# grero/HMMSpikeSorter.jl

Hardware: AMD Instinct MI355X
Metric: Msamples/sec (Viterbi + forward-backward), K=4 L=60 HMM (higher is better)
Workload: dtype f64; 1 GPU; K=4 L=60 HMM (reference N=4, K=60: 237 states), 10000000-sample single channel per GPU: one Viterbi decode + one Baum-Welch E-step (forward-backward + sufficient statistics + M-step finish); channels=1, samples_per_channel=10000000, states=237, engine=wave, block=4928, halo=295, chains=2030, seed=1234, pooled_allreduce=False

## Files before the change

hmmspikesorter.jl_amd/csrc/wave_estep.hip:

```cpp
#include <cmath>
#include <type_traits>

#include "fastmath.h"
#include "wave_common.h"

namespace hmmsort {

constexpr double kLn2 = 6.93147180559945286227e-01;
typedef double wg_d4 __attribute__((ext_vector_type(4)));

__device__ __forceinline__ double scale_of(double v, double s)
{
    return v > 0.0 ? s + (double)ilogb(v) * kLn2 : -INFINITY;
}

template <int N>
struct FIn {
    double y;
    double R[N];
};

template <int N>
__device__ __forceinline__ void excl_sums(const double (&t)[N], double (&out)[N])
{
// ... 82 lines not shown
        d.y = (yc + tb)[li];
#pragma unroll
        for (int a = 0; a < N; a++) d.R[a] = (Rc + (int64_t)a * T + tb)[li];
    };
    int rs = (1 + lane) % RB, ws = (L + 1 + lane) % RB;
    auto run = [&](const FIn<N> &d, int off, auto mode_tag) {
        constexpr int MODE = decltype(mode_tag)::value;
        const int nact = n_total - off < W ? n_total - off : W;
        const bool live = lane < nact;
        const int64_t tb = tinit + 1 + off;
        const int64_t t = tb + lane;
        const double sc0 = KC[0];
        double v[N], E[N + 1];
        double e = -INFINITY;
#pragma unroll
        for (int a = 0; a < N; a++) {
            if (LOGDL) {
                v[a] = 1.0;
                E[a] = live ? DLs[a * (RB + 1) + rs] + sc0 : -INFINITY;
                e = fmax(e, E[a]);
            } else {
                v[a] = live ? DLv[a * (RB + 1) + rs] : 0.0;
                E[a] = DLs[a * (RB + 1) + rs] + sc0;
                e = fmax(e, scale_of(v[a], E[a]));
            }
        }
        const double dd = d.y - KC[1];
        const double q0 = -((dd * dd) * KC[2]);
        float fa = live ? (float)(sc0 + q0) : 0.0f;
        float fb = live ? (float)(e + q0) : -INFINITY;
        scan_maxplus_f32(fa, fb);
        const float Mf = (float)M;
        const float Mtf = fmaxf(Mf + fa, fb);
        const double Mt = (double)Mtf;
        const double Mprev = (double)lane_prevf(Mtf, Mf);
        const double ref = Mt - q0;
        E[N] = (Mprev + sc0) - ref;
#pragma unroll
        for (int a = 0; a < N; a++) E[a] = v[a] > 0.0 ? fmin(E[a] - ref, 700.0) : -INFINITY;
        fexp_n<N + 1>(E);
        const double E0 = E[N];
        double Ea[N];
        double al = E0 * KC[3], be = 0.0;
#pragma unroll
        for (int a = 0; a < N; a++) {
            Ea[a] = LOGDL ? E[a] : v[a] * E[a];
            be = __builtin_fma(Ea[a], KC[KPEND + a], be);
        }
        al = live ? al : 1.0;
        be = live ? be : 0.0;
        scan_linear(al, be);
        const double xt = __builtin_fma(al, x, be);
        const double xprev = lane_prev(xt, x);
        const double einv = KC[4];
        const double base = (xprev * E0) * einv;
        double u[N];
        if (UC) {
            double tb_[N], ex[N];
#pragma unroll
            for (int a = 0; a < N; a++) tb_[a] = Ea[a] * einv;
            excl_sums<N>(tb_, ex);
#pragma unroll
            for (int a = 0; a < N; a++) u[a] = __builtin_fma(ex[a], KC[KCPX + a], base * KC[KCP0 + a]);
        } else {
#pragma unroll
            for (int a = 0; a < N; a++) {
                double su = base * KC[KCP0 + a];
#pragma unroll
                for (int b = 0; b < N; b++)
                    if (b != a) su = __builtin_fma(Ea[b] * einv, KC[KCPX + a * N + b], su);
                u[a] = su;
                __builtin_amdgcn_sched_barrier(0);
            }
        }
        const int wsl = live ? ws : RB;
        if (LOGDL) {
            double lu[N];
#pragma unroll
            for (int a = 0; a < N; a++) lu[a] = u[a];
            flog_n<N>(lu);
#pragma unroll
            for (int a = 0; a < N; a++) DLs[a * (RB + 1) + wsl] = ((ref + KC[KSC + a]) + d.R[a]) + (u[a] > 0.0 ? lu[a] : -INFINITY);
        } else {
#pragma unroll
            for (int a = 0; a < N; a++) {
                DLv[a * (RB + 1) + wsl] = u[a];
                DLs[a * (RB + 1) + wsl] = (ref + KC[KSC + a]) + d.R[a];
            }
        }
        if (MODE == 1) {
            const double la0 = Mt + flog(xt);
            *(live ? FAc + tb + lane : trash + lane) = la0;
            *(live ? FRc + tb + lane : trash + 64 + lane) = ref;
#pragma unroll
            for (int a = 0; a < N; a++) *(live ? FVc + (int64_t)a * T + tb + lane : trash + 64 * (2 + a) + lane) = u[a];
        }
        if (MODE == 2) {
            if (live && t >= tc - L && t < tc) {
                const int64_t jj = t - (tc - L);
#pragma unroll
                for (int a = 0; a < N; a++) rec[1 + jj * (N + 1) + a] = u[a];
                rec[1 + jj * (N + 1) + N] = ref;
                if (t == tc - 1) rec[0] = Mt + flog(xt);
            }
        }
        x = wave_bcast(xt, nact - 1);
        M = wave_bcast(Mt, nact - 1);
        const int ee = x > 0.0 ? ilogb(x) : 0;
        if (ee >= 32 || ee <= -32) {
            const double Mx = M + (double)ee * kLn2, Mn = (double)(float)Mx;
            x = ldexp(x, -ee) * fexp(Mx - Mn);
            M = Mn;
        }
        rs += W; rs = rs >= RB ? rs - RB : rs;
        ws += W; ws = ws >= RB ? ws - RB : ws;
    };
    auto sweep = [&](int from, int to, auto mode_tag) {
        FIn<N> buf[D];
#pragma unroll
        for (int i = 0; i < D; i++) load(buf[i], from + i * W);
        int off = from;
        for (; off + D * W <= to; off += D * W) {
#pragma unroll
            for (int i = 0; i < D; i++) {
                run(buf[i], off + i * W, mode_tag);
                load(buf[i], off + (i + D) * W);
            }
        }
#pragma unroll
        for (int i = 0; i < D; i++)
            if (off + i * W < to) run(buf[i], off + i * W, mode_tag);
    };
    const int n_warm = c == 0 ? 0 : g.Hw - 1;
    const int n_rec = ((L + W - 1) / W) * W < n_warm ? ((L + W - 1) / W) * W : n_warm;
    if (n_warm - n_rec > 0) sweep(0, n_warm - n_rec, std::integral_constant<int, 0>());
    if (n_rec > 0) sweep(n_warm - n_rec, n_warm, std::integral_constant<int, 2>());
    sweep(n_warm, n_total, std::integral_constant<int, 1>());
}

template <int N>
struct BIn {
    double y1, y0;
    double w2;
    double R[N];
    double fv[N];
    double fref, la0;
};

constexpr int bwd_yring(int ft) { return ft <= 2 ? 256 : 512; }

#ifndef HS_BWD_W4
#define HS_BWD_W4 2
#endif
template <int N, bool UC, int FT = 0, bool GS = false>
__global__ __launch_bounds__(64, N <= 4 ? HS_BWD_W4 : 1) void kw_bwd(WaveGeom g, const WaveConst *__restrict__ cst,
                                                            const double *__restrict__ y,
                                                            const double *__restrict__ Rf,
                                                            const double *__restrict__ FA0,
                                                            const double *__restrict__ FV,
                                                            const double *__restrict__ FREF,
                                                            const double *__restrict__ fpre,
                                                            const double *__restrict__ W2,
                                                            double *__restrict__ rho, double *__restrict__ partS,
                                                            double *__restrict__ Zc, double *__restrict__ bpre,
                                                            double *__restrict__ bown, double *__restrict__ yhead,
                                                            double *__restrict__ trash, double *__restrict__ partG,
                                                            double *__restrict__ gsil)
{
    constexpr bool FUSE = FT > 0;
    static_assert(!GS || !FUSE, "the silent posterior is stored by the unfused sweep");
    static_assert(!FUSE || (N >= 3 && N <= 8), "the fused statistics are written for delayed copies of 3-8 rings");
    static_assert(!FUSE || N > 4 || FT == 1, "3-4 rings: one tile of 64 lags");
    constexpr int NPc = N <= 4 ? 4 : 8, NSc = 16 / NPc, LPT = 16 * NSc;
    constexpr int RPAD = NPc == 4 ? 1 : 2;
    constexpr int RGROWS = 128 + 8 * RPAD;
    constexpr int YM = bwd_yring(FT);
    constexpr int NACC = FT <= 1 ? 2 : FT;
#ifndef HS_BWD_D4
#define HS_BWD_D4 2
#endif
    constexpr int D = N <= 4 ? HS_BWD_D4 : (N <= 8 ? 2 : 1);
    constexpr int KSC = 4, KCP0 = 4 + N, KPEND = 4 + 2 * N, KCPX = 4 + 3 * N, KSIZE = 4 + 3 * N + N * N;
    extern __shared__ double lds[];
    const int L = g.L, W = g.W, RB = g.RB, B = g.B;
    double *KC = lds, *DLv = lds + KSIZE, *DLs = lds + KSIZE + N * (RB + 1);
    const int lane = threadIdx.x;
    const int cg = blockIdx.x, ch = cg / g.nch, c = cg % g.nch;
    const int64_t T = g.T;
    const int64_t tc = (int64_t)c * B;
    const int nc = (int)((T - tc) < B ? (T - tc) : B);
    const int64_t tend = tc + nc, tstar = tend - 1;
    const int64_t te = (tend + g.He) < T ? (tend + g.He) : T;
    const double *yc = y + (int64_t)ch * T;
    const double *Rc = Rf + (int64_t)ch * N * T;
    const double *FAc = FA0 + (int64_t)ch * T, *FRc = FREF + (int64_t)ch * T, *FVc = FV + (int64_t)ch * N * T;
    double *rhoc = rho + (int64_t)ch * N * T;
    const double *W2c = W2 + (int64_t)ch * T;
    const int64_t FR = 1 + (int64_t)L * (N + 1);
    const double la0pre = c > 0 ? fpre[cg * FR] : 0.0;
    double *recp = bpre + cg * FR, *reco = bown + cg * FR;
    double *yh = yhead + (int64_t)ch * (N * L + 2);

    for (int i = lane; i < N * (RB + 1); i += 64) DLv[i] = 1.0;
    for (int i = lane; i < RB + 1; i += 64) DLs[i] = 0.0;
    double *YY = DLs + (RB + 1), *RG = YY + YM;
    const int lk = lane >> 4, lj = lane & 15, gla = lj % NPc, glsft = lj / NPc;
    wg_d4 cacc[NACC > 0 ? NACC : 1];
#pragma unroll
    for (int q = 0; q < NACC; q++) cacc[q] = wg_d4{0.0, 0.0, 0.0, 0.0};
    int gtau = -1;
    auto rgrow = [&](int r) { return (r + RPAD * (r >> 4)) * NPc; };
    auto gmfma = [&](int upto) {
        if constexpr (FT <= 1) {
            constexpr int D0 = 16 * (NSc - 1);
            for (; gtau + 8 <= upto; gtau += 8) {
                const int r0 = (gtau + lk - 16 * glsft) & 127, r1 = (gtau + 4 + lk - 16 * glsft) & 127;
                const double b0 = RG[rgrow(r0) + gla], b1 = RG[rgrow(r1) + gla];
                const double a0 = YY[(gtau + lk - D0 - lj) & (YM - 1)], a1 = YY[(gtau + 4 + lk - D0 - lj) & (YM - 1)];
                cacc[0] = __builtin_amdgcn_mfma_f64_16x16x4f64(a0, b0, cacc[0], 0, 0, 0);
                cacc[1] = __builtin_amdgcn_mfma_f64_16x16x4f64(a1, b1, cacc[1], 0, 0, 0);
            }
            if (gtau + 4 <= upto) {
                const int r0 = (gtau + lk - 16 * glsft) & 127;
                const double b0 = RG[rgrow(r0) + gla];
                const double a0 = YY[(gtau + lk - D0 - lj) & (YM - 1)];
                cacc[0] = __builtin_amdgcn_mfma_f64_16x16x4f64(a0, b0, cacc[0], 0, 0, 0);
                gtau += 4;
            }
        } else {
            for (; gtau + 4 <= upto; gtau += 4) {
                const int r0 = (gtau + lk - 16 * glsft) & 127;
                const double b0 = RG[rgrow(r0) + gla];
                double av[FT];
#pragma unroll
                for (int q = 0; q < FT; q++) av[q] = YY[(gtau + lk - (LPT * q + 16 * (NSc - 1)) - lj) & (YM - 1)];
#pragma unroll
                for (int q = 0; q < FT; q++) cacc[q] = __builtin_amdgcn_mfma_f64_16x16x4f64(av[q], b0, cacc[q], 0, 0, 0);
            }
        }
    };
    if (FUSE) {
        for (int i = lane; i < YM + RGROWS * NPc; i += 64) YY[i] = 0.0;
    }
    {
        const WaveConst &Kg = cst[ch];
        if (lane == 0) { KC[0] = Kg.sc0; KC[1] = Kg.mean0; KC[2] = 1.0 / Kg.den; KC[3] = Kg.P00; }
        if (lane < N) { KC[KSC + lane] = Kg.sc[lane]; KC[KCP0 + lane] = Kg.CP0[lane]; KC[KPEND + lane] = Kg.PEND[lane]; }
        if (UC) { if (lane < N) KC[KCPX + lane] = Kg.CPXin[lane]; }
        else for (int i = lane; i < N * N; i += 64) KC[KCPX + i] = Kg.CPX[i];
    }
    __syncthreads();

    double Mb = 0.0, xb = 1.0, z = 0.0;
    double sx[N], ra[N], s2[N], s_all = 0.0, s_m = 0.0, s_y2 = 0.0;
#pragma unroll
    for (int a = 0; a < N; a++) { sx[a] = 0.0; ra[a] = 0.0; s2[a] = 0.0; }

    const int n_warm = (int)(te - tend);
    const int n_total = n_warm + nc;
    const int w0 = n_warm % W ? n_warm % W : W;
    auto start = [&](int k) { return k == 0 ? 0 : w0 + (k - 1) * W; };
    auto width = [&](int done) {
        if (done < n_warm) return done == 0 ? w0 : W;
        return n_total - done < W ? n_total - done : W;
    };
    auto load = [&](BIn<N> &d, int done) {
        const int nact = done < n_total ? width(done) : 0;
        const int li = lane < nact ? lane : 0;
        int64_t tb = te - 2 - done;
        tb = tb < -1 ? -1 : tb;
        const int64_t t = tb - li;
        const int64_t t1 = t + 1 < T ? t + 1 : T - 1;
        const int64_t tz = t < 0 ? 0 : t;
        d.y1 = yc[t1];
        d.y0 = yc[tz];
        d.w2 = W2c[t1];
        d.fref = FRc[t1];
        d.la0 = FAc[tz];
#pragma unroll
        for (int a = 0; a < N; a++) {
            d.R[a] = Rc[(int64_t)a * T + t1];
            d.fv[a] = FVc[(int64_t)a * T + t1];
        }
    };
    auto run = [&](const BIn<N> &d, int done, auto mode_tag) {
        constexpr int MODE = decltype(mode_tag)::value;
        const int nact = width(done);
        const bool live = lane < nact;
        const int64_t tb = te - 2 - done;
        const int64_t t = tb - lane;
        const bool owned = MODE == 1 || MODE == 3 || (MODE == 2 && done >= n_warm);
        if (FUSE) YY[(done + 1 + lane) & (YM - 1)] = d.y1;
        int ws = (done + 1) % RB + lane;
        ws = ws >= RB ? ws - RB : ws;
        int rs = ws - L;
        rs = rs < 0 ? rs + RB : rs;
        const double sc0 = KC[0];
        double vb[N], E[N + 1];
        const double sbv = DLs[rs];
        double e = -INFINITY;
#pragma unroll
        for (int a = 0; a < N; a++) {
            vb[a] = live ? DLv[a * (RB + 1) + rs] : 0.0;
            E[a] = (sbv + d.R[a]) + KC[KSC + a];
            e = fmax(e, scale_of(vb[a], E[a]));
        }
        const double dd = d.y1 - KC[1];
        const double q1 = -((dd * dd) * KC[2]);
        float fa = live ? (float)(q1 + sc0) : 0.0f;
        float fb = live ? (float)e : -INFINITY;
        scan_maxplus_f32(fa, fb);
        const float Mbf = (float)Mb;
        const float Mtf = fmaxf(Mbf + fa, fb);
        const double Mt = (double)Mtf;
        const double Mnext = (double)lane_prevf(Mtf, Mbf);
        E[N] = ((Mnext + q1) + sc0) - Mt;
#pragma unroll
        for (int a = 0; a < N; a++) E[a] = vb[a] > 0.0 ? fmin(E[a] - Mt, 700.0) : -INFINITY;
        fexp_n<N + 1>(E);
        const double E0 = E[N];
        double wa[N];
        double al = E0 * KC[3], be = 0.0;
#pragma unroll
        for (int a = 0; a < N; a++) {
            wa[a] = vb[a] * E[a];
            be = __builtin_fma(wa[a], KC[KCP0 + a], be);
        }
        al = live ? al : 1.0;
        be = live ? be : 0.0;
        scan_linear(al, be);
        const double xt = __builtin_fma(al, xb, be);
        const double xnext = lane_prev(xt, xb);
        const double base = xnext * E0;
        double yn[N];
        if (UC) {
            double tq[N], ex[N];
#pragma unroll
            for (int b = 0; b < N; b++) tq[b] = wa[b] * KC[KCPX + b];
            excl_sums<N>(tq, ex);
#pragma unroll
            for (int a = 0; a < N; a++) yn[a] = __builtin_fma(base, KC[KPEND + a], ex[a]);
        } else {
#pragma unroll
            for (int a = 0; a < N; a++) {
                double su = base * KC[KPEND + a];
#pragma unroll
                for (int b = 0; b < N; b++)
                    if (b != a) su = __builtin_fma(wa[b], KC[KCPX + a * N + b], su);
                yn[a] = su;
                __builtin_amdgcn_sched_barrier(0);
            }
        }
        const int wsl = live ? ws : RB;
#pragma unroll
        for (int a = 0; a < N; a++) DLv[a * (RB + 1) + wsl] = yn[a];
        DLs[wsl] = Mt;
        if (MODE == 2 && live) {
            double *rr = nullptr;
            int64_t jj = 0;
            if (!owned && t >= tend && t < tend + L) { rr = recp; jj = t - tend; }
            if (owned && t >= tc && t < tc + L) { rr = reco; jj = t - tc; }
            if (rr) {
#pragma unroll
                for (int a = 0; a < N; a++) rr[1 + jj * (N + 1) + a] = yn[a];
                rr[1 + jj * (N + 1) + N] = Mt;
                if (jj == 0) rr[0] = Mt + flog(xt);
            }
        }
        if (owned) {
            const double la = t >= tc ? d.la0 : la0pre;
            double gg[2] = {fmin((la + Mt) - z, 700.0), fmin((d.fref + Mt) - z, 700.0)};
            fexp_n<2>(gg);
            const int64_t t1 = t + 1;
            if (live && t >= tc && t >= g.own_lo && t < g.own_hi) {
                const double ga = xt * gg[0];
                s_all += ga;
                if (!g.last || t < T - 1) s_m += ga;
                s_y2 = __builtin_fma(ga, d.y0 * d.y0, s_y2);
            }
            if (GS) *(live && t >= tc ? gsil + (int64_t)ch * T + t : trash + 64 * N + lane) = xt * gg[0];
            const bool own1 = live && t1 >= g.own_lo && t1 < g.own_hi;
            const bool bulk = !(g.last && t1 > T - L);
#pragma unroll
            for (int a = 0; a < N; a++) {
                const double rv = own1 ? (d.fv[a] * wa[a]) * gg[1] : 0.0;
                if (MODE != 3) *(live ? rhoc + (int64_t)a * T + t1 : trash + 64 * a + lane) = rv;
                ra[a] += bulk ? rv : 0.0;
                s2[a] = __builtin_fma(rv, d.w2, s2[a]);
                sx[a] += (own1 && t >= 0) ? wa[a] * gg[0] : 0.0;
                if (FUSE) RG[rgrow((done + 1 + lane) & 127) + a] = rv;
            }
            if (FUSE) {
#pragma unroll
                for (int a = N; a < NPc; a++) RG[rgrow((done + 1 + lane) & 127) + a] = 0.0;
                if (gtau < 0) gtau = (done + 1) & ~3;
                gmfma(done + 1 + nact);
            }
            if (MODE == 2 && c == 0 && t < L && live && t >= 0) {
                double lg[N + 1];
#pragma unroll
                for (int a = 0; a < N; a++) lg[a] = yn[a];
                lg[N] = xt;
                flog_n<N + 1>(lg);
#pragma unroll
                for (int a = 0; a < N; a++) yh[a * L + t] = Mt + lg[a];
                if (t == 0) yh[N * L] = Mt + lg[N];
            }
        }
        xb = wave_bcast(xt, nact - 1);
        Mb = wave_bcast(Mt, nact - 1);
        const int ee = xb > 0.0 ? ilogb(xb) : 0;
        if (ee >= 32 || ee <= -32) {
            const double Mx = Mb + (double)ee * kLn2, Mn = (double)(float)Mx;
            xb = ldexp(xb, -ee) * fexp(Mx - Mn);
            Mb = Mn;
        }
    };
    auto znorm = [&]() {
        __syncthreads();
        const double la = FAc[tstar];
        double zmax = la + Mb + (double)ilogb(xb) * kLn2;
        double sc_[N], mant[N];
        for (int i0 = 0; i0 < L; i0 += 64) {
            const int i = i0 + lane;
            const bool on = i < L;
            const int64_t tp = tstar - (on ? i : 0);
            int slot = (int)((te - 1 - (tp + L - 1)) % RB);
            slot = slot < 0 ? slot + RB : slot;
            const double sbv = DLs[slot], fr = FRc[tp];
#pragma unroll
            for (int a = 0; a < N; a++) {
                const double m = FVc[(int64_t)a * T + tp] * DLv[a * (RB + 1) + slot];
                const double s = ((fr + KC[KSC + a]) + Rc[(int64_t)a * T + tp]) + sbv;
                if (on) zmax = fmax(zmax, scale_of(m, s));
            }
        }
        zmax = wave_max(zmax);
        double zs = 0.0;
        for (int i0 = 0; i0 < L; i0 += 64) {
            const int i = i0 + lane;
            const bool on = i < L;
            const int64_t tp = tstar - (on ? i : 0);
            int slot = (int)((te - 1 - (tp + L - 1)) % RB);
            slot = slot < 0 ? slot + RB : slot;
            const double sbv = DLs[slot], fr = FRc[tp];
#pragma unroll
            for (int a = 0; a < N; a++) {
                mant[a] = FVc[(int64_t)a * T + tp] * DLv[a * (RB + 1) + slot];
                sc_[a] = mant[a] > 0.0 ? fmin((((fr + KC[KSC + a]) + Rc[(int64_t)a * T + tp]) + sbv) - zmax, 700.0) : -INFINITY;
            }
            fexp_n<N>(sc_);
#pragma unroll
            for (int a = 0; a < N; a++) zs += on ? mant[a] * sc_[a] : 0.0;
        }
        zs = wave_sum(zs);
        zs += xb * fexp((la + Mb) - zmax);
        z = zmax + flog(zs);
        if (lane == 0) {
            Zc[cg] = z;
            if (GS) gsil[(int64_t)ch * T + tstar] = xb * fexp((la + Mb) - z);
            if (tstar >= g.own_lo && tstar < g.own_hi) {
                const double ga = xb * fexp((la + Mb) - z);
                s_all += ga;
                if (!g.last || tstar < T - 1) s_m += ga;
                const double yv = yc[tstar];
                s_y2 = __builtin_fma(ga, yv * yv, s_y2);
            }
        }
        __syncthreads();
    };

    const int nsteps = n_total <= 0 ? 0 : 1 + (n_total - w0 + W - 1) / W;
    const int kwarm = n_warm == 0 ? 0 : 1 + (n_warm - w0) / W;
    const int rk = (L + W - 1) / W + 1;
    auto sweep = [&](int k0, int k1, auto mode_tag) {
        BIn<N> buf[D];
#pragma unroll
        for (int i = 0; i < D; i++) load(buf[i], start(k0 + i));
        int k = k0;
        for (; k + D <= k1; k += D) {
#pragma unroll
            for (int i = 0; i < D; i++) {
                run(buf[i], start(k + i), mode_tag);
                load(buf[i], start(k + i + D));
            }
        }
#pragma unroll
        for (int i = 0; i < D; i++)
            if (k + i < k1) run(buf[i], start(k + i), mode_tag);
    };
    const int kw1 = kwarm - rk > 0 ? kwarm - rk : 0;
    if (kw1 > 0) sweep(0, kw1, std::integral_constant<int, 0>());
    if (kwarm > kw1) sweep(kw1, kwarm, std::integral_constant<int, 2>());
    znorm();
    const int ko1 = nsteps - rk > kwarm ? nsteps - rk : kwarm;
    if (FUSE) {
        const int km = kwarm + rk < ko1 ? kwarm + rk : ko1;
        if (km > kwarm) sweep(kwarm, km, std::integral_constant<int, 1>());
        if (ko1 > km) sweep(km, ko1, std::integral_constant<int, 3>());
    } else if (ko1 > kwarm) sweep(kwarm, ko1, std::integral_constant<int, 1>());
    if (nsteps > ko1) sweep(ko1, nsteps, std::integral_constant<int, 2>());
    if (FUSE) {
        const int sig_end = n_total + 1;
        if (gtau >= 0) {
#pragma unroll
            for (int a = 0; a < NPc; a++) RG[rgrow((sig_end + lane) & 127) + a] = 0.0;
            gmfma(sig_end + 16 * (NSc - 1) + 4);
        }
        double *pg = partG + (int64_t)cg * N * L;
#pragma unroll
        for (int q = 0; q < (FT <= 1 ? 1 : FT); q++)
#pragma unroll
            for (int r = 0; r < 4; r++) {
                const int lag = LPT * q + 16 * (NSc - 1 - glsft) + lk + 4 * r;
                const double v = FT <= 1 ? cacc[0][r] + cacc[1][r] : cacc[q][r];
                if (gla < N && lag < L) pg[gla * L + lag] = v;
            }
    }
    double *ps = partS + (int64_t)cg * (3 * N + 3);
#pragma unroll
    for (int a = 0; a < N; a++) {
        const double v1 = wave_sum(sx[a]), v2 = wave_sum(ra[a]), v3 = wave_sum(s2[a]);
        if (lane == 0) { ps[a] = v1; ps[N + a] = v2; ps[2 * N + a] = v3; }
    }
    {
        const double v1 = wave_sum(s_all), v2 = wave_sum(s_m), v3 = wave_sum(s_y2);
        if (lane == 0) { ps[3 * N] = v1; ps[3 * N + 1] = v2; ps[3 * N + 2] = v3; }
    }
}

__global__ __launch_bounds__(64) void kw_fb_check(WaveGeom g, double tol, const double *__restrict__ FA0,
                                                  const double *__restrict__ FV, const double *__restrict__ FREF,
                                                  const double *__restrict__ fpre, const double *__restrict__ bpre,
                                                  const double *__restrict__ bown, const double *__restrict__ rho,
                                                  int64_t *__restrict__ diag, double *__restrict__ dbg)
{
    const int lane = threadIdx.x;
    const int cg = blockIdx.x, ch = cg / g.nch, c = cg % g.nch;
    if (c == 0) return;
    const int N = g.N, L = g.L;
    const int64_t T = g.T, tc = (int64_t)c * g.B;
    const int64_t FR = 1 + (int64_t)L * (N + 1);
    const double *FAc = FA0 + (int64_t)ch * T, *FRc = FREF + (int64_t)ch * T, *FVc = FV + (int64_t)ch * N * T;
    const double *rhoc = rho + (int64_t)ch * N * T;
    for (int dir = 0; dir < 2; dir++) {
        const int ne = dir == 0 ? L : L - 1;
        auto weight = [&](int a, int e) {
            const int64_t tp = dir == 0 ? tc - 1 - e : tc + e - L + 1;
            return tp >= 0 ? rhoc[(int64_t)a * T + tp] : 0.0;
        };
        auto diff = [&](int a, int e) {
            double hv, hs, mv, ms;
            if (dir == 0) {
                const int64_t tp = tc - 1 - e, jj = tp - (tc - L);
                hv = fpre[cg * FR + 1 + jj * (N + 1) + a]; hs = fpre[cg * FR + 1 + jj * (N + 1) + N];
                mv = FVc[(int64_t)a * T + tp]; ms = FRc[tp];
            } else {
                hv = bpre[(cg - 1) * FR + 1 + (int64_t)e * (N + 1) + a]; hs = bpre[(cg - 1) * FR + 1 + (int64_t)e * (N + 1) + N];
                mv = bown[cg * FR + 1 + (int64_t)e * (N + 1) + a]; ms = bown[cg * FR + 1 + (int64_t)e * (N + 1) + N];
            }
            if (hv == mv && hs == ms) return 0.0;
            if (!(hv > 0.0) && !(mv > 0.0)) return 0.0;
            return (hs - ms) + (flog(hv) - flog(mv));
        };
        double ringmass = 0.0;
        const int64_t tb = dir == 0 ? tc - 1 : tc;
        for (int idx = lane; idx < N * L; idx += 64) {
            const int a = idx / L, k = idx % L;
            const int64_t tp = tb - k;
            if (tp >= 0) ringmass += rhoc[(int64_t)a * T + tp];
        }
        ringmass = wave_sum(ringmass);
        const double w0 = fmax(1.0 - ringmass, 0.0);
        const double d0 = dir == 0 ? fpre[cg * FR] - FAc[tc - 1] : bpre[(cg - 1) * FR] - bown[cg * FR];
        double wb = lane == 0 ? w0 : -1.0, db = d0;
        int bi = -1;
        for (int idx = lane; idx < N * ne; idx += 64) {
            const int a = idx / ne, e = idx % ne;
            const double w = weight(a, e);
            if (w > wb) { wb = w; db = diff(a, e); bi = idx; }
        }
        for (int o = 32; o > 0; o >>= 1) {
            const double ow = __shfl_xor(wb, o), od = __shfl_xor(db, o);
            const int oi = __shfl_xor(bi, o);
            if (ow > wb) { wb = ow; db = od; bi = oi; }
        }
        bi = __builtin_amdgcn_readfirstlane(bi);
        const double D = wave_bcast(db, 0);
        double err = lane == 0 ? w0 * fabs(fexp(fmin(d0 - D, 700.0)) - 1.0) : 0.0;
        for (int idx = lane; idx < N * ne; idx += 64) {
            const int a = idx / ne, e = idx % ne;
            const double w = weight(a, e);
            if (w > 0.0) err += w * fabs(fexp(fmin(diff(a, e) - D, 700.0)) - 1.0);
        }
        err = wave_sum(err);
        if (lane == 0) {
            if (!(err <= tol) && dbg && atomicAdd((unsigned long long *)&diag[3 + 2 * dir], 0ull) == 0ull) {
                dbg[0] = cg; dbg[1] = dir; dbg[2] = D; dbg[3] = w0; dbg[4] = d0; dbg[5] = err; dbg[6] = ringmass;
                dbg[7] = wb; dbg[8] = bi; dbg[9] = tc; dbg[10] = ne;
            }
            if (!(err <= tol)) atomicAdd((unsigned long long *)&diag[3 + 2 * dir], 1ull);
            if (err == err) {
                const unsigned long long eb = (unsigned long long)__double_as_longlong(err);
                if (eb > *reinterpret_cast<volatile unsigned long long *>(&diag[4 + 2 * dir]))
                    atomicMax((unsigned long long *)&diag[4 + 2 * dir], eb);
            }
        }
    }
}

constexpr int kGsTile = 4096, kGsSub = 256;

__global__ __launch_bounds__(256) void kw_gsum_generic(WaveGeom g, const double *__restrict__ y,
                                                       const double *__restrict__ rho, int nparts,
                                                       double *__restrict__ partG)
{
    extern __shared__ double lds[];
    const int N = g.N, L = g.L, NL = N * L, ch = blockIdx.y;
    double *lr = lds;
    double *ly = lds + N * kGsSub;
    const int64_t T = g.T, t0 = (int64_t)blockIdx.x * kGsTile;
    const double *yc = y + (int64_t)ch * T, *rc = rho + (int64_t)ch * N * T;
    const int p = threadIdx.x + 256 * blockIdx.z;
    const int a = p < NL ? p / L : 0, k = p < NL ? p % L : 0;
    double s1 = 0.0;
    for (int s0 = 0; s0 < kGsTile; s0 += kGsSub) {
        const int64_t tb = t0 + s0;
        if (tb >= T) break;
        __syncthreads();
        for (int i = threadIdx.x; i < N * kGsSub; i += 256) {
            const int aa = i / kGsSub, u = i % kGsSub;
            const int64_t t = tb + u;
            lr[i] = t < T ? rc[(int64_t)aa * T + t] : 0.0;
        }
        for (int i = threadIdx.x; i < kGsSub + L; i += 256) {
            const int64_t t = tb + i;
            ly[i] = t < T ? yc[t] : 0.0;
        }
        __syncthreads();
#pragma unroll 4
        for (int u = 0; u < kGsSub; u++) {
            const double r = lr[a * kGsSub + u], yv = ly[u + k];
            s1 = __builtin_fma(r, yv, s1);
        }
    }
    double *out = partG + ((int64_t)ch * nparts + blockIdx.x) * NL;
    if (p < NL) out[p] = s1;
}

constexpr int kGxTR = 64, kGxBv = 512, kGxSubs = 1;

template <int N, int NT>
__global__ __launch_bounds__(256) void kw_gsum_mx(WaveGeom g, const double *__restrict__ y,
                                                  const double *__restrict__ rho, int nparts,
                                                  double *__restrict__ partG)
{
    constexpr int NP = N <= 1 ? 1 : (N <= 2 ? 2 : (N <= 4 ? 4 : (N <= 8 ? 8 : 16)));
    constexpr int NS = 16 / NP, LPT = 16 * NS, HS = 16 * (NS - 1);
    constexpr int TR = kGxTR, CW = 8, RR = TR + HS, Bv = kGxBv;
// ... 72 lines not shown
                    const double a = lyc[ts * 4 + q * LPT];
                    c1[q] = __builtin_amdgcn_mfma_f64_16x16x4f64(a, b, c1[q], 0, 0, 0);
                }
            }
        }
    }
    const int NL = N * L;
    double *out = partG + ((int64_t)ch * nparts + blockIdx.x) * NL;
    double *red = lds;
#pragma unroll
    for (int q = 0; q < NT; q++) {
        __syncthreads();
#pragma unroll
        for (int r = 0; r < 4; r++) red[(wv * 4 + r) * 64 + lane] = c1[q][r];
        __syncthreads();
        {
            const int e = tid;
            const int ln = e & 63, r = e >> 6;
            double v = 0.0;
#pragma unroll
            for (int w = 0; w < 4; w++) v += red[(w * 4 + r) * 64 + ln];
            const int j = ln & 15, a = j % NP, sft = j / NP;
            const int lag = lag0 + q * LPT + 16 * sft + (ln >> 4) + 4 * r;
            if (a < N && lag < L) out[a * L + lag] = v;
        }
    }
}

__global__ __launch_bounds__(64) void kw_stats_final(WaveGeom g, int rowsG, const double *__restrict__ partG,
                                                     const double *__restrict__ partS, const double *__restrict__ y,
                                                     const double *__restrict__ Rf, const double *__restrict__ virt,
                                                     const double *__restrict__ FA0, const double *__restrict__ rho,
                                                     const double *__restrict__ Zc, const double *__restrict__ yhead,
                                                     double *__restrict__ pp, double *__restrict__ stats)
{
    const int N = g.N, L = g.L, i = blockIdx.x, ch = blockIdx.y, lane = threadIdx.x;
    const int NL = N * L, ws = 3 * N + 3, total = 3 * NL + N + 4, S = 1 + NL;
    const double *pS = partS + (int64_t)ch * g.nch * ws;
    const double *pG = partG + (int64_t)ch * rowsG * NL;
    auto colsum = [&](const double *p, int rows, size_t stride) {
        double a0 = 0.0, a1 = 0.0, a2 = 0.0, a3 = 0.0, a4 = 0.0, a5 = 0.0, a6 = 0.0, a7 = 0.0;
        int r = lane;
        for (; r + 448 < rows; r += 512) {
            a0 += p[(size_t)r * stride];         a1 += p[(size_t)(r + 64) * stride];
            a2 += p[(size_t)(r + 128) * stride]; a3 += p[(size_t)(r + 192) * stride];
            a4 += p[(size_t)(r + 256) * stride]; a5 += p[(size_t)(r + 320) * stride];
            a6 += p[(size_t)(r + 384) * stride]; a7 += p[(size_t)(r + 448) * stride];
        }
        for (; r < rows; r += 64) a0 += p[(size_t)r * stride];
        return ((a0 + a1) + (a2 + a3)) + ((a4 + a5) + (a6 + a7));
    };
    double acc = 0.0;
    if (i < NL) {
        acc = colsum(pS + N + i / L, g.nch, ws);
    } else if (i < 2 * NL) {
        acc = colsum(pG + (i - NL), rowsG, NL);
    } else if (i < 3 * NL) {
        const int e = i - 2 * NL;
        if (e % L == 0) acc = colsum(pS + 2 * N + e / L, g.nch, ws);
    } else if (i < 3 * NL + N) {
        acc = colsum(pS + (i - 3 * NL), g.nch, ws);
    } else if (i < 3 * NL + N + 3) {
        acc = colsum(pS + 3 * N + (i - 3 * NL - N), g.nch, ws);
    }
    if (i < 3 * NL) {
        const int64_t T = g.T;
        const int pair = i % NL, which = i / NL, a = pair / L, k = pair % L + 1;
        const double *yc = y + (int64_t)ch * T, *rc = rho + (int64_t)ch * N * T;
        const double *yh = yhead + (int64_t)ch * (NL + 2);
        const double *V = virt + ((int64_t)ch * N + a) * (L + 1);
        const double z = Zc[(int64_t)ch * g.nch];
        if (g.first)
            for (int j = 1 + lane; j <= L - 1; j += 64) {
                const int idx = -j + k - 1;
                if (idx < 0) continue;
                const double rv = fexp((V[j] + yh[a * L + (L - 1 - j)]) - z);
                const double yv = yc[idx];
                acc += which == 0 ? rv : (which == 1 ? rv * yv : rv * (yv * yv));
            }
        if (which == 0) {
            if (g.last)
                for (int64_t t = T - L + 1 + lane; t <= T - k; t += 64)
                    if (t >= 0) acc += rc[(int64_t)a * T + t];
            if (lane == 0) {
                const double lpv = k == 1 ? Rf[((int64_t)ch * N + a) * T] : V[k - 1];
                pp[(int64_t)ch * S + 1 + pair] = (lpv + yh[a * L + (L - k)]) - z;
                if (pair == 0) pp[(int64_t)ch * S] = (FA0[(int64_t)ch * T] + yh[NL]) - z;
            }
        }
    }
    acc = wave_sum(acc);
    if (lane == 0) stats[(int64_t)ch * total + i] = acc;
}

__global__ __launch_bounds__(256) void kw_mstep(WaveGeom g, const WaveConst *__restrict__ cst,
                                                const double *__restrict__ stats_all,
                                                const double *__restrict__ pp_all, double *__restrict__ out_all)
{
    __shared__ double red[8];
    const int N = g.N, L = g.L, NL = N * L, K = L + 1, ch = blockIdx.x, S = 1 + NL;
    const double *stats = stats_all + (int64_t)ch * (3 * NL + N + 4);
    const double *pp = pp_all + (int64_t)ch * S;
    double *out = out_all + (int64_t)ch * (K * N + 1 + N + S);
    const double *G0 = stats, *G1 = stats + NL, *G2 = stats + 2 * NL, *Xi = stats + 3 * NL;
    const double s_all = stats[3 * NL + N], s_m = stats[3 * NL + N + 1], s_y2 = stats[3 * NL + N + 2];
    double x2 = 0.0, qq = 0.0;
    for (int p = threadIdx.x; p < NL; p += blockDim.x) {
        const int a = p / L, k = p % L + 1;
        const double mu = G1[p] / G0[p];
        out[k + K * a] = mu;
        x2 += (G2[p] - (2.0 * mu) * G1[p]) + (mu * mu) * G0[p];
        qq += G0[p];
    }
    for (int a = threadIdx.x; a < N; a += blockDim.x) {
        out[K * a] = 0.0;
        out[K * N + 1 + a] = (cst[ch].xishift[a] + flog(Xi[a])) - flog(s_m);
    }
    for (int j = threadIdx.x; j < S; j += blockDim.x) out[K * N + 1 + N + j] = pp[j];
    x2 = wave_sum(x2); qq = wave_sum(qq);
    if ((threadIdx.x & 63) == 0) { red[threadIdx.x >> 6] = x2; red[4 + (threadIdx.x >> 6)] = qq; }
    __syncthreads();
    if (threadIdx.x == 0) {
        const double X2 = ((red[0] + red[1]) + (red[2] + red[3])) + s_y2;
        const double QQ = ((red[4] + red[5]) + (red[6] + red[7])) + s_all;
        out[K * N] = sqrt(X2 / QQ);
    }
}

template <typename Kern>
static int wave_lds_attr2(Kern kern, size_t lds)
{
    if (lds > 64 * 1024)
        HS_HIP(hipFuncSetAttribute((const void *)kern, hipFuncAttributeMaxDynamicSharedMemorySize, (int)lds));
    return HMMSORT_OK;
}

static int wave_estep_sweeps(WaveDev *r, const double *d_y, double *d_stats, hipStream_t st, bool wait_cert = true)
{
    const WaveGeom &g = r->g;
    const int N = g.N, L = g.L, NL = N * L;
    const int nchT = g.C * g.nch;
    if (!r->keep_post) r->post_valid = false;
    int rowsG = 0;
    const WavePick p = wave_pick(r, r->keep_post ? kWaveCallPosteriors : kWaveCallEstep);
    int rc = dispatch_N(N, [&](auto n) {
        constexpr int NN = decltype(n)::value;
        const size_t ldsf = ((size_t)(p.logdl ? 1 : 2) * NN * (g.RB + 1) + 5 + 3 * NN + NN * NN) * sizeof(double);
        const bool generic = p.gsum == kGsumGeneric;
        constexpr bool kFuse4 = NN == 3 || NN == 4, kFuse8 = NN >= 5 && NN <= 8;
        const int ft = p.ft;
        HS_CHECK(p.logdl == (NN > 8) && (ft == 0 || (kFuse4 && ft == 1) || (kFuse8 && p.uc && (ft == 2 || ft == 4))),
                 HMMSORT_EINVAL, "wave E-step: no kernel for the picked row (ft %d)", ft);
        const bool fuse = ft > 0;
        const int ym = bwd_yring(ft);
        const size_t ldsb = ((size_t)(NN + 1) * (g.RB + 1) + 4 + 3 * NN + NN * NN +
                             (fuse ? ym + (128 + 8 * (NN <= 4 ? 1 : 2)) * (NN <= 4 ? 4 : 8) : 0)) * sizeof(double);
        auto kf = kw_fwd<NN, true>;
        auto kb = kw_bwd<NN, true>;
        if constexpr (NN <= kWaveMaxPerSource) {
            if (!p.uc) { kf = kw_fwd<NN, false>; kb = kw_bwd<NN, false>; }
        }
        if (p.gs) {
            kb = kw_bwd<NN, true, 0, true>;
            if constexpr (NN <= kWaveMaxPerSource) {
                if (!p.uc) kb = kw_bwd<NN, false, 0, true>;
            }
        }
        if constexpr (kFuse4) {
            if (ft == 1) kb = p.uc ? kw_bwd<NN, true, 1> : kw_bwd<NN, false, 1>;
        }
        if constexpr (kFuse8) {
            if (ft == 2) kb = kw_bwd<NN, true, 2>;
            if (ft == 4) kb = kw_bwd<NN, true, 4>;
        }
        int rc2;
        if ((rc2 = wave_lds_attr2(kf, ldsf)) || (rc2 = wave_lds_attr2(kb, ldsb))) return rc2;
        { WPROF(r, "kw_fwd", st);
          hipLaunchKernelGGL(kf, dim3(nchT), dim3(64), ldsf, st, g, r->d_cst, d_y, r->Rf, r->virt, r->FA0,
                             r->FV, r->FREF, r->fpre, r->trash); }
        { WPROF(r, r->keep_post ? "kw_bwd_post" : "kw_bwd", st);
          hipLaunchKernelGGL(kb, dim3(nchT), dim3(64), ldsb, st, g, r->d_cst, d_y, r->Rf, r->FA0, r->FV,
                             r->FREF, r->fpre, r->W2, r->rho, r->partS, r->Zc, r->bpre, r->bown, r->yhead, r->trash, r->partG,
                             r->gsil); }
        HS_HIP(hipGetLastError());
        HS_HIP(hipEventRecord(r->ev_a, st));
        HS_HIP(hipStreamWaitEvent(r->side, r->ev_a, 0));
        if (g.nch > 1) {
            WPROF(r, "kw_fb_check", r->side);
            hipLaunchKernelGGL(kw_fb_check, dim3(nchT), dim3(64), 0, r->side, g, 1e-9, r->FA0, r->FV, r->FREF, r->fpre,
                               r->bpre, r->bown, r->rho, r->diag, r->dbg);
        }
        HS_HIP(hipEventRecord(r->ev_c, r->side));
        if (r->keep_post) return HMMSORT_OK;
        constexpr int NPx = NN <= 1 ? 1 : (NN <= 2 ? 2 : (NN <= 4 ? 4 : (NN <= 8 ? 8 : 16)));
        constexpr int LPTx = 16 * (16 / NPx), HSx = LPTx - 16;
        if (fuse) {
            rowsG = g.nch;
        } else if (!generic) {
            const int ntk = p.nt, ngrp = p.ngrp;
            HS_CHECK(p.gsum == kGsumMx && ngrp >= 1 && (NN > 8 ? (ntk == 4 || ntk == 8 || ntk == 16) : (ntk >= 1 && ntk <= 4)) &&
                     (int64_t)ntk * ngrp * LPTx >= L, HMMSORT_EINVAL, "wave E-step: no statistics kernel with %d tiles", ntk);
            rowsG = (int)((g.T + kGxSubs * 8 * (int64_t)kGxBv - 1) / (kGxSubs * 8 * (int64_t)kGxBv));
            constexpr int RRx = kGxTR + HSx, RRPx = RRx + RRx / 16 + 1;
            const size_t l1 = ((size_t)8 * (RRPx * NPx + 2) + (size_t)8 * (kGxTR + 19 + LPTx * (ntk - 1))) * 8;
            const size_t l2 = (size_t)4 * 4 * 64 * 8;
            const size_t lds = l1 > l2 ? l1 : l2;
            auto go = [&](auto kern) -> int {
                int rc3 = wave_lds_attr2(kern, lds);
                if (rc3) return rc3;
                WPROF(r, "kw_gsum", st);
                hipLaunchKernelGGL(kern, dim3(rowsG, g.C, ngrp), dim3(256), lds, st, g, d_y, r->rho, rowsG, r->partG);
                return HMMSORT_OK;
            };
            if constexpr (NN > 8) rc2 = ntk == 4 ? go(kw_gsum_mx<NN, 4>) : ntk == 8 ? go(kw_gsum_mx<NN, 8>) : go(kw_gsum_mx<NN, 16>);
            else rc2 = ntk == 1 ? go(kw_gsum_mx<NN, 1>) : ntk == 2 ? go(kw_gsum_mx<NN, 2>)
                       : ntk == 3 ? go(kw_gsum_mx<NN, 3>) : go(kw_gsum_mx<NN, 4>);
            if (rc2) return rc2;
        } else {
            rowsG = r->gparts;
            const size_t lds = ((size_t)NN * kGsSub + kGsSub + L) * sizeof(double);
            WPROF(r, "kw_gsum", st);
            hipLaunchKernelGGL(kw_gsum_generic, dim3(rowsG, g.C, (NL + 255) / 256), dim3(256), lds, st, g, d_y, r->rho, rowsG, r->partG);
        }
        HS_HIP(hipGetLastError());
        return HMMSORT_OK;
    });
    if (rc) return rc;
    if (r->keep_post) {
        HS_HIP(hipStreamWaitEvent(st, r->ev_c, 0));
        return HMMSORT_OK;
    }
    const int total = 3 * NL + N + 4;
    { WPROF(r, "kw_stats_final", st);
      hipLaunchKernelGGL(kw_stats_final, dim3(total, g.C), dim3(64), 0, st, g, rowsG, r->partG, r->partS, d_y, r->Rf,
                         r->virt, r->FA0, r->rho, r->Zc, r->yhead, r->pp, d_stats); }
    if (wait_cert) HS_HIP(hipStreamWaitEvent(st, r->ev_c, 0));
    HS_HIP(hipGetLastError());
    return HMMSORT_OK;
}

int wave_estep(WaveDev *r, const double *d_y, double *d_stats, hipStream_t st)
{
    r->post_valid = false;
    return wave_graphed(r, 2, d_y, d_stats, nullptr, nullptr, st, [&](hipStream_t s) -> int {
        int rc;
        HS_HIP(hipMemsetAsync(r->diag, 0, 8 * sizeof(int64_t), s));
        if ((rc = wave_prepare(r, d_y, s))) return rc;
        return wave_estep_sweeps(r, d_y, d_stats, s);
    });
}

int wave_post_sweeps(WaveDev *r, const double *d_y, hipStream_t st)
{
    int rc;
    HS_HIP(hipMemsetAsync(r->diag, 0, 8 * sizeof(int64_t), st));
    if ((rc = wave_prepare(r, d_y, st))) return rc;
    r->keep_post = true;
    rc = wave_estep_sweeps(r, d_y, nullptr, st);
    r->keep_post = false;
    return rc;
}

int wave_mstep(WaveDev *r, const double *d_stats, double *d_out, hipStream_t st)
{
    { WPROF(r, "kw_mstep", st);
      hipLaunchKernelGGL(kw_mstep, dim3(r->g.C), dim3(256), 0, st, r->g, r->d_cst, d_stats, r->pp, d_out); }
    HS_HIP(hipGetLastError());
    return HMMSORT_OK;
}

int wave_decode_estep(WaveDev *r, const double *d_y, int16_t *d_x, double *d_ll, double *d_stats, hipStream_t st)
{
    r->post_valid = false;
    return wave_graphed(r, 3, d_y, d_x, d_ll, d_stats, st, [&](hipStream_t s) -> int {
        int rc;
        HS_HIP(hipMemsetAsync(r->diag, 0, wave_zero_bytes(r, true), s));
        if ((rc = wave_prepare(r, d_y, s))) return rc;
        HS_HIP(hipEventRecord(r->ev_fork, s));
        HS_HIP(hipStreamWaitEvent(r->side2, r->ev_fork, 0));
        if ((rc = wave_estep_sweeps(r, d_y, d_stats, s, false))) return rc;
        if ((rc = wave_viterbi_sweep(r, d_y, r->side2))) return rc;
        if ((rc = wave_viterbi_post(r, d_y, d_x, d_ll, r->side2, true))) return rc;
        HS_HIP(hipEventRecord(r->ev_join, r->side2));
        HS_HIP(hipStreamWaitEvent(s, r->ev_join, 0));
        HS_HIP(hipStreamWaitEvent(s, r->ev_c, 0));
        return HMMSORT_OK;
    });
}

}
```

Baseline: 10600 Msamples/s.

## Add interior sweep mode and mirrored LDS rings to fused backward kernel

The fused backward kernel (FT==1, N<=4) now keeps mirrored copies of the y and rho rings in LDS. The MFMA feed loop can then address them through fixed per-lane base pointers with one wrap computation, instead of recomputing masked indices for every operand. It also adds an interior sweep mode for steps fully inside the owned range. That mode uses unpredicated strided loads, drops the ownership/boundary predicates, and skips the rho global store. The cost is extra LDS for the mirror regions and duplicate stores on each ring write, plus more complex range bookkeeping for the interior steps.

```diff
diff --git a/hmmspikesorter.jl_amd/csrc/wave_estep.hip b/hmmspikesorter.jl_amd/csrc/wave_estep.hip
--- a/hmmspikesorter.jl_amd/csrc/wave_estep.hip
+++ b/hmmspikesorter.jl_amd/csrc/wave_estep.hip
@@ -258,6 +258,28 @@
 #ifndef HS_BWD_W4
 #define HS_BWD_W4 2
 #endif
+#ifndef HS_BWD_FEED
+#define HS_BWD_FEED 1
+#endif
+#ifndef HS_BWD_ILOAD
+#define HS_BWD_ILOAD 1
+#endif
+#ifndef HS_BWD_IPRED
+#define HS_BWD_IPRED 1
+#endif
+constexpr int bwd_np(int n) { return n <= 4 ? 4 : 8; }
+constexpr int bwd_d0(int n) { return 16 * (16 / bwd_np(n) - 1); }
+constexpr int bwd_ymir(int n) { return bwd_d0(n) + 20; }
+constexpr int bwd_rmir(int n) { return bwd_d0(n); }
+constexpr bool bwd_feed(int ft) { return HS_BWD_FEED && ft == 1; }
+constexpr int bwd_stat_doubles(int n, int ft)
+{
+    const int np = bwd_np(n), rpad = n <= 4 ? 1 : 2, ym = bwd_yring(ft);
+    if (ft <= 0) return 0;
+    if (!bwd_feed(ft)) return ym + (128 + 8 * rpad) * np;
+    const int re = 128 + bwd_rmir(n);
+    return (ym + bwd_ymir(n) + 2) + (re + rpad * (re >> 4) + 1) * np;
+}
 template <int N, bool UC, int FT = 0, bool GS = false>
 __global__ __launch_bounds__(64, N <= 4 ? HS_BWD_W4 : 1) void kw_bwd(WaveGeom g, const WaveConst *__restrict__ cst,
                                                             const double *__restrict__ y,
@@ -277,7 +299,7 @@
     static_assert(!GS || !FUSE, "the silent posterior is stored by the unfused sweep");
     static_assert(!FUSE || (N >= 3 && N <= 8), "the fused statistics are written for delayed copies of 3-8 rings");
     static_assert(!FUSE || N > 4 || FT == 1, "3-4 rings: one tile of 64 lags");
-    constexpr int NPc = N <= 4 ? 4 : 8, NSc = 16 / NPc, LPT = 16 * NSc;
+    constexpr int NPc = bwd_np(N), NSc = 16 / NPc, LPT = 16 * NSc;
     constexpr int RPAD = NPc == 4 ? 1 : 2;
     constexpr int RGROWS = 128 + 8 * RPAD;
     constexpr int YM = bwd_yring(FT);
@@ -309,15 +331,55 @@
 
     for (int i = lane; i < N * (RB + 1); i += 64) DLv[i] = 1.0;
     for (int i = lane; i < RB + 1; i += 64) DLs[i] = 0.0;
-    double *YY = DLs + (RB + 1), *RG = YY + YM;
+    double *YY = DLs + (RB + 1), *RG = YY + (bwd_feed(FT) ? YM + bwd_ymir(N) + 2 : YM);
     const int lk = lane >> 4, lj = lane & 15, gla = lj % NPc, glsft = lj / NPc;
     wg_d4 cacc[NACC > 0 ? NACC : 1];
 #pragma unroll
     for (int q = 0; q < NACC; q++) cacc[q] = wg_d4{0.0, 0.0, 0.0, 0.0};
     int gtau = -1;
     auto rgrow = [&](int r) { return (r + RPAD * (r >> 4)) * NPc; };
+    constexpr bool FEED = bwd_feed(FT);
+    constexpr int YMIR = bwd_ymir(N), RMIR = bwd_rmir(N), RE = 128 + RMIR;
+    const double *RGl = RG + (rgrow(lk - 16 * glsft + RMIR) + gla);
+    const double *YYl = YY + (lk - lj + (YMIR - 16 * (NSc - 1) - 4));
+    auto ystore = [&](int sigma, double v) {
+        const int i = sigma & (YM - 1);
+        if constexpr (FEED) {
+            YY[YMIR + i] = v;
+            YY[i >= YM - YMIR ? i - (YM - YMIR) : YM + YMIR] = v;
+        } else YY[i] = v;
+    };
+    auto rstore = [&](int sigma, const double (&v)[NPc]) {
+        const int r = sigma & 127;
+        if constexpr (FEED) {
+            double *p0 = RG + rgrow(RMIR + r), *p1 = RG + rgrow(r >= 128 - RMIR ? r - (128 - RMIR) : RE);
+#pragma unroll
+            for (int a = 0; a < NPc; a++) p0[a] = v[a];
+#pragma unroll
+            for (int a = 0; a < NPc; a++) p1[a] = v[a];
+        } else {
+            double *p0 = RG + rgrow(r);
+#pragma unroll
+            for (int a = 0; a < NPc; a++) p0[a] = v[a];
+        }
+    };
     auto gmfma = [&](int upto) {
-        if constexpr (FT <= 1) {
+        if constexpr (FEED) {
+            for (; gtau + 8 <= upto; gtau += 8) {
+                const int s0 = rgrow(gtau & 127), s1 = rgrow((gtau + 4) & 127), sy = (gtau + 4) & (YM - 1);
+                const double b0 = RGl[s0], b1 = RGl[s1];
+                const double a0 = YYl[sy], a1 = YYl[sy + 4];
+                cacc[0] = __builtin_amdgcn_mfma_f64_16x16x4f64(a0, b0, cacc[0], 0, 0, 0);
+                cacc[1] = __builtin_amdgcn_mfma_f64_16x16x4f64(a1, b1, cacc[1], 0, 0, 0);
+            }
+            if (gtau + 4 <= upto) {
+                const int s0 = rgrow(gtau & 127), sy = (gtau + 4) & (YM - 1);
+                const double b0 = RGl[s0];
+                const double a0 = YYl[sy];
+                cacc[0] = __builtin_amdgcn_mfma_f64_16x16x4f64(a0, b0, cacc[0], 0, 0, 0);
+                gtau += 4;
+            }
+        } else if constexpr (FT <= 1) {
             constexpr int D0 = 16 * (NSc - 1);
             for (; gtau + 8 <= upto; gtau += 8) {
                 const int r0 = (gtau + lk - 16 * glsft) & 127, r1 = (gtau + 4 + lk - 16 * glsft) & 127;
@@ -346,7 +408,8 @@
         }
     };
     if (FUSE) {
-        for (int i = lane; i < YM + RGROWS * NPc; i += 64) YY[i] = 0.0;
+        static_assert(!FUSE || FEED || bwd_stat_doubles(N, FT) == YM + RGROWS * NPc, "the launch sizes the rings with bwd_stat_doubles");
+        for (int i = lane; i < bwd_stat_doubles(N, FT); i += 64) YY[i] = 0.0;
     }
     {
         const WaveConst &Kg = cst[ch];
@@ -370,7 +433,24 @@
         if (done < n_warm) return done == 0 ? w0 : W;
         return n_total - done < W ? n_total - done : W;
     };
-    auto load = [&](BIn<N> &d, int done) {
+    int imax = 0;
+    const unsigned ivo = (unsigned)(W - 1 - (lane < W ? lane : 0)) & 63u;
+    auto load = [&](BIn<N> &d, int done, auto mode_tag) {
+        if constexpr (decltype(mode_tag)::value == 4 && HS_BWD_ILOAD) {
+            const int dn = done < imax ? done : imax;
+            const int64_t t0 = te - 1 - dn - W;
+            d.y1 = (yc + t0 + 1)[ivo];
+            d.y0 = (yc + t0)[ivo];
+            d.w2 = (W2c + t0 + 1)[ivo];
+            d.fref = (FRc + t0 + 1)[ivo];
+            d.la0 = (FAc + t0)[ivo];
+#pragma unroll
+            for (int a = 0; a < N; a++) {
+                d.R[a] = (Rc + (int64_t)a * T + t0 + 1)[ivo];
+                d.fv[a] = (FVc + (int64_t)a * T + t0 + 1)[ivo];
+            }
+            return;
+        }
         const int nact = done < n_total ? width(done) : 0;
         const int li = lane < nact ? lane : 0;
         int64_t tb = te - 2 - done;
@@ -391,12 +471,13 @@
     };
     auto run = [&](const BIn<N> &d, int done, auto mode_tag) {
         constexpr int MODE = decltype(mode_tag)::value;
-        const int nact = width(done);
+        constexpr bool IPRED = MODE == 4 && HS_BWD_IPRED;
+        const int nact = MODE == 4 ? W : width(done);
         const bool live = lane < nact;
         const int64_t tb = te - 2 - done;
         const int64_t t = tb - lane;
-        const bool owned = MODE == 1 || MODE == 3 || (MODE == 2 && done >= n_warm);
-        if (FUSE) YY[(done + 1 + lane) & (YM - 1)] = d.y1;
+        const bool owned = MODE == 1 || MODE == 3 || MODE == 4 || (MODE == 2 && done >= n_warm);
+        if (FUSE) ystore(done + 1 + lane, d.y1);
         int ws = (done + 1) % RB + lane;
         ws = ws >= RB ? ws - RB : ws;
         int rs = ws - L;
@@ -474,31 +555,34 @@
             }
         }
         if (owned) {
-            const double la = t >= tc ? d.la0 : la0pre;
+            const double la = (IPRED || t >= tc) ? d.la0 : la0pre;
             double gg[2] = {fmin((la + Mt) - z, 700.0), fmin((d.fref + Mt) - z, 700.0)};
             fexp_n<2>(gg);
             const int64_t t1 = t + 1;
-            if (live && t >= tc && t >= g.own_lo && t < g.own_hi) {
+            const bool osil = IPRED ? live : (live && t >= tc && t >= g.own_lo && t < g.own_hi);
+            if (osil) {
                 const double ga = xt * gg[0];
                 s_all += ga;
-                if (!g.last || t < T - 1) s_m += ga;
+                if (IPRED || !g.last || t < T - 1) s_m += ga;
                 s_y2 = __builtin_fma(ga, d.y0 * d.y0, s_y2);
             }
             if (GS) *(live && t >= tc ? gsil + (int64_t)ch * T + t : trash + 64 * N + lane) = xt * gg[0];
-            const bool own1 = live && t1 >= g.own_lo && t1 < g.own_hi;
-            const bool bulk = !(g.last && t1 > T - L);
+            const bool own1 = IPRED ? live : (live && t1 >= g.own_lo && t1 < g.own_hi);
+            const bool bulk = IPRED || !(g.last && t1 > T - L);
+            double rvv[NPc];
 #pragma unroll
             for (int a = 0; a < N; a++) {
                 const double rv = own1 ? (d.fv[a] * wa[a]) * gg[1] : 0.0;
-                if (MODE != 3) *(live ? rhoc + (int64_t)a * T + t1 : trash + 64 * a + lane) = rv;
+                if (MODE != 3 && MODE != 4) *(live ? rhoc + (int64_t)a * T + t1 : trash + 64 * a + lane) = rv;
                 ra[a] += bulk ? rv : 0.0;
                 s2[a] = __builtin_fma(rv, d.w2, s2[a]);
-                sx[a] += (own1 && t >= 0) ? wa[a] * gg[0] : 0.0;
-                if (FUSE) RG[rgrow((done + 1 + lane) & 127) + a] = rv;
+                sx[a] += (own1 && (IPRED || t >= 0)) ? wa[a] * gg[0] : 0.0;
+                if (a < NPc) rvv[a] = rv;
             }
             if (FUSE) {
 #pragma unroll
-                for (int a = N; a < NPc; a++) RG[rgrow((done + 1 + lane) & 127) + a] = 0.0;
+                for (int a = N; a < NPc; a++) rvv[a] = 0.0;
+                rstore(done + 1 + lane, rvv);
                 if (gtau < 0) gtau = (done + 1) & ~3;
                 gmfma(done + 1 + nact);
             }
@@ -582,13 +666,13 @@
     auto sweep = [&](int k0, int k1, auto mode_tag) {
         BIn<N> buf[D];
 #pragma unroll
-        for (int i = 0; i < D; i++) load(buf[i], start(k0 + i));
+        for (int i = 0; i < D; i++) load(buf[i], start(k0 + i), mode_tag);
         int k = k0;
         for (; k + D <= k1; k += D) {
 #pragma unroll
             for (int i = 0; i < D; i++) {
                 run(buf[i], start(k + i), mode_tag);
-                load(buf[i], start(k + i + D));
+                load(buf[i], start(k + i + D), mode_tag);
             }
         }
 #pragma unroll
@@ -603,14 +687,35 @@
     if (FUSE) {
         const int km = kwarm + rk < ko1 ? kwarm + rk : ko1;
         if (km > kwarm) sweep(kwarm, km, std::integral_constant<int, 1>());
-        if (ko1 > km) sweep(km, ko1, std::integral_constant<int, 3>());
+        int ki0 = ko1, ki1 = ko1;
+        if constexpr (HS_BWD_ILOAD || HS_BWD_IPRED) {
+            const int64_t ohi = g.own_hi < tend ? g.own_hi : tend, olo = g.own_lo > tc ? g.own_lo : tc;
+            int64_t dlo = te - ohi, dhi = te - 1 - W - olo;
+            if (g.last && dlo < te - 1 - (T - L)) dlo = te - 1 - (T - L);
+            if (dhi >= dlo && dhi >= 0) {
+                const int x0 = (int)dlo - w0, x1 = (int)dhi - w0;
+                const int k0i = x0 > 0 ? 1 + (x0 + W - 1) / W : (x0 > -W ? 1 : 0);
+                const int k1i = x1 >= 0 ? 2 + x1 / W : (x1 >= -W ? 1 : 0);
+                ki0 = k0i > km ? k0i : km;
+                ki1 = k1i < ko1 ? k1i : ko1;
+                if (ki1 <= ki0) ki0 = ki1 = ko1;
+            }
+        }
+        if (ki0 > km) sweep(km, ki0, std::integral_constant<int, 3>());
+        if (ki1 > ki0) {
+            imax = start(ki1 - 1);
+            sweep(ki0, ki1, std::integral_constant<int, 4>());
+        }
+        if (ko1 > ki1) sweep(ki1, ko1, std::integral_constant<int, 3>());
     } else if (ko1 > kwarm) sweep(kwarm, ko1, std::integral_constant<int, 1>());
     if (nsteps > ko1) sweep(ko1, nsteps, std::integral_constant<int, 2>());
     if (FUSE) {
         const int sig_end = n_total + 1;
         if (gtau >= 0) {
-#pragma unroll
-            for (int a = 0; a < NPc; a++) RG[rgrow((sig_end + lane) & 127) + a] = 0.0;
+            double zero[NPc];
+#pragma unroll
+            for (int a = 0; a < NPc; a++) zero[a] = 0.0;
+            rstore(sig_end + lane, zero);
             gmfma(sig_end + 16 * (NSc - 1) + 4);
         }
         double *pg = partG + (int64_t)cg * N * L;
@@ -989,9 +1094,7 @@
         HS_CHECK(p.logdl == (NN > 8) && (ft == 0 || (kFuse4 && ft == 1) || (kFuse8 && p.uc && (ft == 2 || ft == 4))),
                  HMMSORT_EINVAL, "wave E-step: no kernel for the picked row (ft %d)", ft);
         const bool fuse = ft > 0;
-        const int ym = bwd_yring(ft);
-        const size_t ldsb = ((size_t)(NN + 1) * (g.RB + 1) + 4 + 3 * NN + NN * NN +
-                             (fuse ? ym + (128 + 8 * (NN <= 4 ? 1 : 2)) * (NN <= 4 ? 4 : 8) : 0)) * sizeof(double);
+        const size_t ldsb = ((size_t)(NN + 1) * (g.RB + 1) + 4 + 3 * NN + NN * NN + bwd_stat_doubles(NN, ft)) * sizeof(double);
         auto kf = kw_fwd<NN, true>;
         auto kb = kw_bwd<NN, true>;
         if constexpr (NN <= kWaveMaxPerSource) {
```

After: 10920 Msamples/s (median of 6 runs). 1.03x the previous value.
